# anonyomous4/parallel-c-programs

Measured on AMD Instinct MI355X. Metric: TFLOPS SGEMM 8192^2 + GB/s reduce 1e9 f32, at 1/2/4/8 MI355X, higher is better.
Workload: dtype fp32; 1 GPU; global_batch=1, parallelism=dp1

## Files before the change

### csrc/kernels/sgemm_x6.hip

```cpp
#include "pcmx_common.h"
#include "pcmx_hip.h"
#include <type_traits>

namespace {
typedef float f32x16 __attribute__((ext_vector_type(16)));
typedef __bf16 bf16x8 __attribute__((ext_vector_type(8)));
typedef __bf16 bf16x2 __attribute__((ext_vector_type(2)));
typedef float f32x2 __attribute__((ext_vector_type(2)));
typedef unsigned u32x4 __attribute__((ext_vector_type(4)));
using pcmx::f32x4;

struct Planes {
    u32x4 p[3];
};

__device__ __forceinline__ unsigned cvt2(float a, float b) {
    const f32x2 v = {a, b};
    return __builtin_bit_cast(unsigned, __builtin_convertvector(v, bf16x2));
}
__device__ __forceinline__ float lo16(unsigned w) { return __uint_as_float(w << 16); }
__device__ __forceinline__ float hi16(unsigned w) { return __uint_as_float(w & 0xffff0000u); }

template <bool FAKE = false>
__device__ __forceinline__ void split_a4(f32x4 (&r)[2], Planes& o) {
#pragma unroll
    for (int q = 0; q < 2; ++q) {
        f32x2 x0 = {r[q][0], r[q][1]}, x1 = {r[q][2], r[q][3]};
#pragma unroll
        for (int l = 0; l < 3; ++l) {
            if (FAKE && l > 0) {
                o.p[l][2 * q] = o.p[0][2 * q], o.p[l][2 * q + 1] = o.p[0][2 * q + 1];
                continue;
            }
            const unsigned w0 = cvt2(x0[0], x0[1]), w1 = cvt2(x1[0], x1[1]);
            o.p[l][2 * q] = w0, o.p[l][2 * q + 1] = w1;
            if (!FAKE && l < 2) x0 -= f32x2{lo16(w0), hi16(w0)}, x1 -= f32x2{lo16(w1), hi16(w1)};
        }
    }
}
template <bool FAKE = false>
__device__ __forceinline__ void split_b_word(const f32x4 (&r)[8], int d, Planes (&o)[4]) {
    f32x2 x[2][2];
#pragma unroll
    for (int e = 0; e < 2; ++e)
#pragma unroll
        for (int jp = 0; jp < 2; ++jp) x[e][jp] = f32x2{r[2 * d + e][2 * jp], r[2 * d + e][2 * jp + 1]};
#pragma unroll
    for (int l = 0; l < 3; ++l) {
        unsigned w[4];
        if (FAKE && l > 0) {
#pragma unroll
            for (int j = 0; j < 4; ++j) o[j].p[l][d] = o[j].p[0][d];
            continue;
        }
#pragma unroll
        for (int j = 0; j < 4; ++j) o[j].p[l][d] = w[j] = cvt2(x[0][j >> 1][j & 1], x[1][j >> 1][j & 1]);
        if (!FAKE && l < 2) {
#pragma unroll
            for (int jp = 0; jp < 2; ++jp) {
                x[0][jp] -= f32x2{lo16(w[2 * jp]), lo16(w[2 * jp + 1])};
                x[1][jp] -= f32x2{hi16(w[2 * jp]), hi16(w[2 * jp + 1])};
            }
        }
    }
}

constexpr int kPA[6] = {2, 1, 0, 1, 0, 0};
constexpr int kPB[6] = {0, 1, 2, 0, 1, 0};

__device__ __forceinline__ f32x16 mfma(const u32x4& a, const u32x4& b, const f32x16& c) {
    return __builtin_amdgcn_mfma_f32_32x32x16_bf16(__builtin_bit_cast(bf16x8, a), __builtin_bit_cast(bf16x8, b), c, 0,
                                                   0, 0);
}

template <bool BETA, int VPM>
__global__ __launch_bounds__(256, 1) void sgemm_x6_kernel(const float* __restrict__ A, const float* __restrict__ B,
                                                          float* __restrict__ C, int M, int N, int K, int lda, int ldb,
                                                          int ldc, float alpha, float beta) {
    const int lane = pcmx::lane_id();
    const int wave = __builtin_amdgcn_readfirstlane(threadIdx.x >> 6);
    const int wm = wave >> 1, wn = wave & 1;
    const int h = lane >> 5, l32 = lane & 31;
    const int tiles_m = M / 256, tiles_n = N / 256;
    const int t = pcmx::xcd_remap((int)blockIdx.x, tiles_m * tiles_n);
    const int per_group = 8 * tiles_n, first_m = (t / per_group) * 8;
    const int gsz = min(tiles_m - first_m, 8);
    const int m0 = __builtin_amdgcn_readfirstlane((first_m + (t % per_group) % gsz) * 256);
    const int n0 = __builtin_amdgcn_readfirstlane(((t % per_group) / gsz) * 256);

    const __amdgpu_buffer_rsrc_t rA = __builtin_amdgcn_make_buffer_rsrc((void*)A, (short)0, 0x7fffffff, 0x00020000);
    const __amdgpu_buffer_rsrc_t rB = __builtin_amdgcn_make_buffer_rsrc((void*)B, (short)0, 0x7fffffff, 0x00020000);
    const __amdgpu_buffer_rsrc_t rC = __builtin_amdgcn_make_buffer_rsrc((void*)C, (short)0, 0x7fffffff, 0x00020000);
    int voA[4];
#pragma unroll
    for (int i = 0; i < 4; ++i) voA[i] = ((32 * i + l32) * lda + 8 * h) * 4;
    const int voB = (8 * h * ldb + 4 * l32) * 4;
    const int voC = (4 * h * ldc + 4 * l32) * 4;
    const int ab = __builtin_amdgcn_readfirstlane((m0 + wm * 128) * lda * 4);
    const int bb = __builtin_amdgcn_readfirstlane((n0 + wn * 128) * 4);
    const int ns = K / 16, last = ns - 1;
    const int bstep = ldb * 64;
    auto ld = [](__amdgpu_buffer_rsrc_t r, int vo, int so) {
        return __builtin_bit_cast(f32x4, __builtin_amdgcn_raw_buffer_load_b128(r, vo, so, 0));
    };
    auto load_a = [&](f32x4 (&dst)[2], int i, int s) __attribute__((always_inline)) {
        const int so = ab + min(s, last) * 64;
        dst[0] = ld(rA, voA[i], so);
        dst[1] = ld(rA, voA[i] + 16, so);
    };
    auto load_b = [&](f32x4 (&dst)[8], int s) __attribute__((always_inline)) {
        const int so = bb + min(s, last) * bstep;
#pragma unroll
        for (int e = 0; e < 8; ++e) dst[e] = ld(rB, voB, so + e * ldb * 4);
    };

    f32x4 ra[4][2];
    f32x4 rb[2][8];
    Planes pa[2];
    Planes pb[2][4];
    f32x16 acc[4][4];
#pragma unroll
    for (int i = 0; i < 4; ++i)
#pragma unroll
        for (int j = 0; j < 4; ++j) acc[i][j] = f32x16{0};

    load_a(ra[0], 0, 0);
    load_b(rb[0], 0);
#pragma unroll
    for (int d = 0; d < 4; ++d) split_b_word(rb[0], d, pb[0]);
    split_a4(ra[0], pa[0]);
    __builtin_amdgcn_sched_barrier(0);
    load_b(rb[1], 1);
#pragma unroll
    for (int i = 1; i < 4; ++i) load_a(ra[i], i, 0);
    load_a(ra[0], 0, 1);
    load_b(rb[0], 2);
    __builtin_amdgcn_sched_barrier(0);

    auto step = [&](int s, auto P_) __attribute__((always_inline)) {
        constexpr int P = decltype(P_)::value;
#pragma unroll
        for (int i = 0; i < 4; ++i) {
            __builtin_amdgcn_sched_barrier(0);
            const Planes& cur = pa[i & 1];
            const int in = (i + 1) & 3;
            split_a4<(VPM >= 10)>(ra[in], pa[in & 1]);
            load_a(ra[in], in, i < 3 ? s + 1 : s + 2);
            split_b_word<(VPM >= 10)>(rb[P ^ 1], i, pb[P ^ 1]);
            if (i == 3) load_b(rb[P ^ 1], s + 3);
#pragma unroll
            for (int p = 0; p < 6; ++p)
#pragma unroll
                for (int j = 0; j < 4; ++j) acc[i][j] = mfma(cur.p[kPA[p]], pb[P][j].p[kPB[p]], acc[i][j]);
            if constexpr (VPM % 10 > 0) {
#pragma unroll
                for (int m = 0; m < 24; ++m) {
                    __builtin_amdgcn_sched_group_barrier(0x008, 1, 0);
                    __builtin_amdgcn_sched_group_barrier(0x002, VPM % 10, 0);
                }
            }
        }
    };
    for (int s = 0; s < ns; s += 2) {
        step(s, std::integral_constant<int, 0>{});
        step(s + 1, std::integral_constant<int, 1>{});
    }

    const int r0 = m0 + wm * 128, c0 = n0 + wn * 128;
#pragma unroll
    for (int i = 0; i < 4; ++i)
#pragma unroll
        for (int r = 0; r < 16; ++r) {
            const int so = ((r0 + i * 32 + (r & 3) + 8 * (r >> 2)) * ldc + c0) * 4;
            f32x4 v{alpha * acc[i][0][r], alpha * acc[i][1][r], alpha * acc[i][2][r], alpha * acc[i][3][r]};
            if constexpr (BETA) v += beta * ld(rC, voC, so);
            __builtin_amdgcn_raw_buffer_store_b128(__builtin_bit_cast(u32x4, v), rC, voC, so, 0);
            __builtin_amdgcn_sched_barrier(0);
        }
}
}

namespace {
template <class F>
int launch_x6(const float* A, const float* B, float* C, int M, int N, int K, int lda, int ldb, int ldc, F&& go) {
    if (M <= 0 || N <= 0 || K <= 0 || M % 256 || N % 256 || K % 32) return PCMX_ERR_ARG;
    if ((lda | ldb | ldc) & 3 || (((uintptr_t)A | (uintptr_t)B | (uintptr_t)C) & 15)) return PCMX_ERR_ARG;
    if ((long long)M * lda * 4 >= (1LL << 31) || (long long)K * ldb * 4 >= (1LL << 31) ||
        (long long)M * ldc * 4 >= (1LL << 31))
        return PCMX_ERR_ARG;
    go((M / 256) * (N / 256));
    return (int)hipGetLastError();
}
}

extern "C" int pcmx_sgemm_f32_x6_variant(const float* A, const float* B, float* C, int M, int N, int K, int lda,
                                         int ldb, int ldc, float alpha, float beta, int v, hipStream_t s) {
    return launch_x6(A, B, C, M, N, K, lda, ldb, ldc, [&](int tiles) {
#define PCMX_X6(VPM)                                                                                                  \
    (beta != 0.f                                                                                                      \
         ? sgemm_x6_kernel<true, VPM><<<tiles, 256, 0, s>>>(A, B, C, M, N, K, lda, ldb, ldc, alpha, beta)             \
         : sgemm_x6_kernel<false, VPM><<<tiles, 256, 0, s>>>(A, B, C, M, N, K, lda, ldb, ldc, alpha, beta))
        switch (v) {
            case 2: PCMX_X6(2); break;
            case 4: PCMX_X6(4); break;
            case 5: PCMX_X6(0); break;
            case 13: PCMX_X6(13); break;
            default: PCMX_X6(3); break;
        }
#undef PCMX_X6
    });
}

extern "C" int pcmx_sgemm_f32_x6(const float* A, const float* B, float* C, int M, int N, int K, int lda, int ldb,
                                 int ldc, float alpha, float beta, hipStream_t s) {
    return pcmx_sgemm_f32_x6_variant(A, B, C, M, N, K, lda, ldb, ldc, alpha, beta, 0, s);
}
```

Measured before the change: 153.9 TFLOPS.

## Interleave bf16 split ops and staggered loads one-by-one between MFMAs

Adds a PACED kernel path, now the default, that breaks the fp32-to-bf16x3 split of A and B into 88 scalar micro-ops. These ops are scheduled explicitly between the 24 MFMAs of each step using sched_barriers. B is loaded row by row into a single buffer instead of double-buffered whole tiles, and global loads are spread at fixed MFMA slots. The aim is to hide split VALU work and load issue under the MFMA stream while cutting register pressure. It drops the old VPM variants, and its rigid hand scheduling could serialize poorly or add instruction overhead.

```diff
diff --git a/csrc/kernels/sgemm_x6.hip b/csrc/kernels/sgemm_x6.hip
--- a/csrc/kernels/sgemm_x6.hip
+++ b/csrc/kernels/sgemm_x6.hip
@@ -1,6 +1,7 @@
 #include "pcmx_common.h"
 #include "pcmx_hip.h"
 #include <type_traits>
+#include <utility>
 
 namespace {
 typedef float f32x16 __attribute__((ext_vector_type(16)));
@@ -73,7 +74,51 @@
                                                    0, 0);
 }
 
-template <bool BETA, int VPM>
+struct Split8 {
+    float x[16];
+    float t[16];
+};
+constexpr int kSplitOps = 88;
+
+__device__ __forceinline__ void put_word(int l, int p, unsigned w, Planes& oa, Planes (&ob)[4], int d) {
+    if (p < 4)
+        oa.p[l][p] = w;
+    else
+        ob[p - 4].p[l][d] = w;
+}
+__device__ __forceinline__ float sub_scalar(float a, float b) {
+    float r = a - b;
+    asm volatile("" : "+v"(r));
+    return r;
+}
+__device__ __forceinline__ float cvt1(float x) { return __uint_as_float(cvt2(0.f, x)); }
+__device__ __forceinline__ unsigned pack_hi(float lo, float hi) {
+    return __builtin_amdgcn_perm(__float_as_uint(hi), __float_as_uint(lo), 0x07060302u);
+}
+
+template <int N>
+__device__ __forceinline__ void split_op(Split8& s, Planes& oa, Planes (&ob)[4], int d) {
+    constexpr int R = N % 40, L = N / 40;
+    if constexpr (L == 2) {
+        put_word(2, R, pack_hi(s.x[2 * R], s.x[2 * R + 1]), oa, ob, d);
+    } else if constexpr (R < 16) {
+        s.t[R] = cvt1(s.x[R]);
+    } else if constexpr (R < 32) {
+        s.x[R - 16] = sub_scalar(s.x[R - 16], s.t[R - 16]);
+    } else {
+        put_word(L, R - 32, pack_hi(s.t[2 * (R - 32)], s.t[2 * (R - 32) + 1]), oa, ob, d);
+    }
+}
+
+constexpr int ops_before(int g) { return 4 * g - 2 * ((g > 11) + (g > 14) + (g > 17) + (g > 20)); }
+static_assert(ops_before(24) == kSplitOps);
+
+template <class F, int... I>
+__device__ __forceinline__ void static_for(std::integer_sequence<int, I...>, F&& f) {
+    (f(std::integral_constant<int, I>{}), ...);
+}
+
+template <bool BETA, bool PACED, bool FAKE>
 __global__ __launch_bounds__(256, 1) void sgemm_x6_kernel(const float* __restrict__ A, const float* __restrict__ B,
                                                           float* __restrict__ C, int M, int N, int K, int lda, int ldb,
                                                           int ldc, float alpha, float beta) {
@@ -113,9 +158,12 @@
 #pragma unroll
         for (int e = 0; e < 8; ++e) dst[e] = ld(rB, voB, so + e * ldb * 4);
     };
+    auto load_b_row = [&](f32x4& dst, int e, int s) __attribute__((always_inline)) {
+        dst = ld(rB, voB, bb + min(s, last) * bstep + e * ldb * 4);
+    };
 
     f32x4 ra[4][2];
-    f32x4 rb[2][8];
+    f32x4 rb[PACED ? 1 : 2][8];
     Planes pa[2];
     Planes pb[2][4];
     f32x16 acc[4][4];
@@ -130,11 +178,20 @@
     for (int d = 0; d < 4; ++d) split_b_word(rb[0], d, pb[0]);
     split_a4(ra[0], pa[0]);
     __builtin_amdgcn_sched_barrier(0);
-    load_b(rb[1], 1);
-#pragma unroll
-    for (int i = 1; i < 4; ++i) load_a(ra[i], i, 0);
-    load_a(ra[0], 0, 1);
-    load_b(rb[0], 2);
+    if constexpr (!PACED) {
+        load_b(rb[1], 1);
+#pragma unroll
+        for (int i = 1; i < 4; ++i) load_a(ra[i], i, 0);
+        load_a(ra[0], 0, 1);
+        load_b(rb[0], 2);
+    } else {
+#pragma unroll
+        for (int i = 0; i < 4; ++i) {
+            load_a(ra[(i + 1) & 3], (i + 1) & 3, i < 3 ? 0 : 1);
+            load_b_row(rb[0][2 * i], 2 * i, 1);
+            load_b_row(rb[0][2 * i + 1], 2 * i + 1, 1);
+        }
+    }
     __builtin_amdgcn_sched_barrier(0);
 
     auto step = [&](int s, auto P_) __attribute__((always_inline)) {
@@ -144,20 +201,43 @@
             __builtin_amdgcn_sched_barrier(0);
             const Planes& cur = pa[i & 1];
             const int in = (i + 1) & 3;
-            split_a4<(VPM >= 10)>(ra[in], pa[in & 1]);
-            load_a(ra[in], in, i < 3 ? s + 1 : s + 2);
-            split_b_word<(VPM >= 10)>(rb[P ^ 1], i, pb[P ^ 1]);
-            if (i == 3) load_b(rb[P ^ 1], s + 3);
-#pragma unroll
-            for (int p = 0; p < 6; ++p)
-#pragma unroll
-                for (int j = 0; j < 4; ++j) acc[i][j] = mfma(cur.p[kPA[p]], pb[P][j].p[kPB[p]], acc[i][j]);
-            if constexpr (VPM % 10 > 0) {
+            if constexpr (!PACED) {
+                split_a4<FAKE>(ra[in], pa[in & 1]);
+                load_a(ra[in], in, i < 3 ? s + 1 : s + 2);
+                split_b_word<FAKE>(rb[P ^ 1], i, pb[P ^ 1]);
+                if (i == 3) load_b(rb[P ^ 1], s + 3);
+#pragma unroll
+                for (int p = 0; p < 6; ++p)
+#pragma unroll
+                    for (int j = 0; j < 4; ++j) acc[i][j] = mfma(cur.p[kPA[p]], pb[P][j].p[kPB[p]], acc[i][j]);
 #pragma unroll
                 for (int m = 0; m < 24; ++m) {
                     __builtin_amdgcn_sched_group_barrier(0x008, 1, 0);
-                    __builtin_amdgcn_sched_group_barrier(0x002, VPM % 10, 0);
+                    __builtin_amdgcn_sched_group_barrier(0x002, 3, 0);
                 }
+            } else {
+                Split8 st;
+#pragma unroll
+                for (int q = 0; q < 2; ++q)
+#pragma unroll
+                    for (int e = 0; e < 4; ++e) st.x[4 * q + e] = ra[in][q][e];
+#pragma unroll
+                for (int j = 0; j < 4; ++j) st.x[8 + 2 * j] = rb[0][2 * i][j], st.x[9 + 2 * j] = rb[0][2 * i + 1][j];
+                const int sa = i < 3 ? s + 1 : s + 2;
+                static_for(std::make_integer_sequence<int, 24>{}, [&](auto G_) __attribute__((always_inline)) {
+                    constexpr int g = decltype(G_)::value, j = g & 3, p = g >> 2;
+                    constexpr int o0 = ops_before(g), o1 = ops_before(g + 1);
+                    acc[i][j] = mfma(cur.p[kPA[p]], pb[P][j].p[kPB[p]], acc[i][j]);
+                    __builtin_amdgcn_sched_barrier(0);
+                    static_for(std::make_integer_sequence<int, o1 - o0>{}, [&](auto O_) __attribute__((always_inline)) {
+                        split_op<o0 + decltype(O_)::value>(st, pa[in & 1], pb[P ^ 1], i);
+                    });
+                    if constexpr (g == 11) ra[in][0] = ld(rA, voA[in], ab + min(sa, last) * 64);
+                    if constexpr (g == 14) ra[in][1] = ld(rA, voA[in] + 16, ab + min(sa, last) * 64);
+                    if constexpr (g == 17) load_b_row(rb[0][2 * i], 2 * i, s + 2);
+                    if constexpr (g == 20) load_b_row(rb[0][2 * i + 1], 2 * i + 1, s + 2);
+                    __builtin_amdgcn_sched_barrier(0);
+                });
             }
         }
     };
@@ -196,16 +276,14 @@
 extern "C" int pcmx_sgemm_f32_x6_variant(const float* A, const float* B, float* C, int M, int N, int K, int lda,
                                          int ldb, int ldc, float alpha, float beta, int v, hipStream_t s) {
     return launch_x6(A, B, C, M, N, K, lda, ldb, ldc, [&](int tiles) {
-#define PCMX_X6(VPM)                                                                                                  \
+#define PCMX_X6(...)                                                                                                  \
     (beta != 0.f                                                                                                      \
-         ? sgemm_x6_kernel<true, VPM><<<tiles, 256, 0, s>>>(A, B, C, M, N, K, lda, ldb, ldc, alpha, beta)             \
-         : sgemm_x6_kernel<false, VPM><<<tiles, 256, 0, s>>>(A, B, C, M, N, K, lda, ldb, ldc, alpha, beta))
+         ? sgemm_x6_kernel<true, __VA_ARGS__><<<tiles, 256, 0, s>>>(A, B, C, M, N, K, lda, ldb, ldc, alpha, beta)     \
+         : sgemm_x6_kernel<false, __VA_ARGS__><<<tiles, 256, 0, s>>>(A, B, C, M, N, K, lda, ldb, ldc, alpha, beta))
         switch (v) {
-            case 2: PCMX_X6(2); break;
-            case 4: PCMX_X6(4); break;
-            case 5: PCMX_X6(0); break;
-            case 13: PCMX_X6(13); break;
-            default: PCMX_X6(3); break;
+            case 1: PCMX_X6(false, false); break;
+            case 13: PCMX_X6(false, true); break;
+            default: PCMX_X6(true, false); break;
         }
 #undef PCMX_X6
     });
```

New measurement: 153.9 TFLOPS (median of 2 runs). No clear change (-0.0%).
